# Oreoluwa-Se/Lidar-Imu-Slam

Measured on NVIDIA B200. Metric: deskew+ICP+GN-loop odometry throughput at 128k pts/scan, higher is better.
Workload: dtype f64

## Files before the change

### lidar-imu-slam_b200/csrc/voxelize.cu

```cuda
#include <algorithm>

#include "compact.cuh"
#include "grid_sync.cuh"
#include "imu_compensate.cuh"
#include "ops.cuh"
#include "voxel_map.cuh"

LIMU_TRACE_RING(limu_debug_trace_vox)

namespace limu {

constexpr int VX_BLOCK = 1024;
constexpr int VX_RUNS = 64;

struct VoxelizeArgs {
    const void *raw;
    const double *ts;
    int mode, stride, deskew;
    double twist[6];
    const double *twist_dev;
    int64_t n;
    double vs1, vs2;
    double *frame, *down, *src0;
    unsigned long long *keys1, *keys2;
    unsigned int *min1, *min2, *pslot1, *pslot2;
    unsigned long long *keys2_prev;
    unsigned int *min2_prev, *pslot2_prev;
    int *nd_prev, *nd_this;
    unsigned int mask1, mask2;
    int shift1, shift2;
    unsigned long long *tile1, *tile2;
    unsigned int epoch;
    int *counts;
    unsigned int *barrier;
    DevStatus *st;
    DevStatus *st_next;
};
struct VoxelizeImuArgs : VoxelizeArgs {
    ImuDeskew imu;
};

__device__ __forceinline__ unsigned int claim(unsigned long long *keys, unsigned int *minidx, int shift, unsigned int mask, const V3 &p, double vs,
                                              unsigned int index, DevStatus *st) {
    const int kx = vox_index(p.x, vs), ky = vox_index(p.y, vs), kz = vox_index(p.z, vs);
    if (!key_in_range(kx, ky, kz)) { st->key_range = 1; return PEND_NONE; }
    const unsigned long long key = pack_key(kx, ky, kz);
    unsigned int s = slot_of(key, shift);
    for (unsigned int probes = 0; probes <= mask; ++probes) {
        const unsigned long long cur = atomicCAS(&keys[s], KEY_EMPTY, key);
        if (cur == KEY_EMPTY || cur == key) { atomicMin(&minidx[s], index); return s; }
        s = (s + 1) & mask;
    }
    st->table_full = 1;
    return PEND_NONE;
}

__device__ __forceinline__ int block_exclusive_scan_count(int c, int *total, int *warp_sums ) {
    const int lane = threadIdx.x & 31, warp = threadIdx.x >> 5;
    int incl = c;
#pragma unroll
    for (int o = 1; o < 32; o <<= 1) { const int t = __shfl_up_sync(0xFFFFFFFFu, incl, o); if (lane >= o) incl += t; }
    if (lane == 31) warp_sums[warp] = incl;
    __syncthreads();
    if (warp == 0) {
        const int nw = (blockDim.x + 31) >> 5;
        const int v = lane < nw ? warp_sums[lane] : 0;
        int wi = v;
#pragma unroll
        for (int o = 1; o < 32; o <<= 1) { const int t = __shfl_up_sync(0xFFFFFFFFu, wi, o); if (lane >= o) wi += t; }
        warp_sums[lane] = wi - v;
        if (lane == 31) *total = wi;
    }
    __syncthreads();
    return warp_sums[warp] + incl - c;
}

template <int BLOCK>
__device__ __forceinline__ int tile_base(const unsigned long long *words, int tile, unsigned int epoch, int *ws ) {
    int part = 0;
    for (int b = threadIdx.x; b < tile; b += BLOCK) {
        unsigned long long w;
        do {
            asm volatile("ld.relaxed.gpu.global.u64 %0, [%1];" : "=l"(w) : "l"(words + b) : "memory");
        } while ((unsigned int)(w >> 32) != epoch);
        part += (int)(unsigned int)w;
    }
#pragma unroll
    for (int o = 16; o > 0; o >>= 1) part += __shfl_down_sync(0xFFFFFFFFu, part, o);
    __syncthreads();
    if ((threadIdx.x & 31) == 0) ws[threadIdx.x >> 5] = part;
    __syncthreads();
    int v = 0;
#pragma unroll
    for (int w = 0; w < BLOCK / 32; ++w) v += ws[w];
    __syncthreads();
    return v;
}
__device__ __forceinline__ void tile_publish(unsigned long long *word, unsigned int epoch, int count) {
    asm volatile("st.relaxed.gpu.global.u64 [%0], %1;" ::"l"(word), "l"(((unsigned long long)epoch << 32) | (unsigned int)count) : "memory");
}

#ifdef LIMU_ICP_PHASE_TIMING
__device__ unsigned long long g_vox_marks[8];
#define VX_MARK(k) do { if (blockIdx.x == 0 && threadIdx.x == 0) { unsigned long long _t; asm volatile("mov.u64 %0, %%globaltimer;" : "=l"(_t)); g_vox_marks[k] = _t; } } while (0)
#else
#define VX_MARK(k) do {} while (0)
#endif

__device__ __forceinline__ Pose deskew_motion(double t, const double *tw) {
    const double s = t - 0.5;
    double st[6];
#pragma unroll
    for (int k = 0; k < 6; ++k) st[k] = s * tw[k];
    return se3_exp(st);
}

template <bool IMU, class Args>
__device__ __forceinline__ void voxelize_body(const Args &A) {
    __shared__ int ws[32];
    __shared__ int total;
    GridSync gs{A.barrier, 0u, gridDim.x};
    const int64_t n = A.n;
    const int64_t gtid = (int64_t)blockIdx.x * VX_BLOCK + threadIdx.x, gthreads = (int64_t)gridDim.x * VX_BLOCK;
    const int ntiles = (int)((n + VX_BLOCK - 1) / VX_BLOCK);
    VX_MARK(0);
    LIMU_TRACE(10);
    {
        const int ndp = __ldcg(A.nd_prev);
        for (int64_t j = gtid; j < ndp; j += gthreads) {
            const unsigned int sl = __ldcg(A.pslot2_prev + j);
            if (sl != PEND_NONE) { A.keys2_prev[sl] = KEY_EMPTY; A.min2_prev[sl] = PEND_NONE; }
        }
    }
    if constexpr (IMU) {
        for (int64_t i = gtid; i < n; i += gthreads) {
            const unsigned char *r = static_cast<const unsigned char *>(A.raw) + (size_t)i * A.stride;
            const float *q = reinterpret_cast<const float *>(r);
            float xyz[3] = {q[0], q[1], q[2]};
            imu_deskew_point(A.imu.table, A.imu.M, i, imu_point_time(r, A.imu.toff), A.imu.rot_end, A.imu.pos_lidar_end, A.imu.p_il, xyz);
            const V3 p{(double)xyz[0], (double)xyz[1], (double)xyz[2]};
            A.frame[3 * i] = p.x; A.frame[3 * i + 1] = p.y; A.frame[3 * i + 2] = p.z;
            A.pslot1[i] = claim(A.keys1, A.min1, A.shift1, A.mask1, p, A.vs1, (unsigned int)i, A.st);
        }
    } else {
        __shared__ double tw[6];
        if (A.deskew && threadIdx.x == 0) {
#pragma unroll
            for (int k = 0; k < 6; ++k) tw[k] = A.twist_dev ? __ldcg(A.twist_dev + k) : A.twist[k];
        }
        __shared__ unsigned long long last_t[VX_BLOCK / 32];
        __shared__ Pose runs[VX_RUNS];
        const int lane = threadIdx.x & 31, warp = threadIdx.x >> 5;
        for (int tile = blockIdx.x; tile < ntiles; tile += gridDim.x) {
            const int64_t i = (int64_t)tile * VX_BLOCK + threadIdx.x;
            const bool live = i < n;
            double t = 0.0;
            if (live && A.deskew) t = A.mode == 0 ? (double)__ldg(reinterpret_cast<const float4 *>(A.raw) + i).w : A.mode == 1 ? A.ts[i] : 0.0;
            Pose T{};
            if (A.deskew) {
                const unsigned long long tb = (unsigned long long)__double_as_longlong(t);
                unsigned long long prev = __shfl_up_sync(0xFFFFFFFFu, tb, 1);
                if (lane == 31) last_t[warp] = tb;
                __syncthreads();
                if (lane == 0 && warp > 0) prev = last_t[warp - 1];
                const int head = live && (threadIdx.x == 0 || tb != prev);
                const int run = block_exclusive_scan_count(head, &total, ws) + head - 1;
                const bool table = total <= VX_RUNS;
                if (table && head) runs[run].qx = t;
                if (table) __syncthreads();
                const bool mine = table ? (int)threadIdx.x < total : live;
                if (mine) T = deskew_motion(table ? runs[threadIdx.x].qx : t, tw);
                if (table) {
                    if (mine) runs[threadIdx.x] = T;
                    __syncthreads();
                    if (live) T = runs[run];
                }
            }
            if (live) {
                V3 p;
                if (A.mode == 0) {
                    const float4 q = __ldg(reinterpret_cast<const float4 *>(A.raw) + i);
                    p = V3{(double)q.x, (double)q.y, (double)q.z};
                } else if (A.mode == 1) {
                    const float *q = reinterpret_cast<const float *>(static_cast<const unsigned char *>(A.raw) + (size_t)i * A.stride);
                    p = V3{(double)q[0], (double)q[1], (double)q[2]};
                } else {
                    const double *q = static_cast<const double *>(A.raw) + 3 * i;
                    p = V3{q[0], q[1], q[2]};
                }
                if (A.deskew) p = apply(T, p);
                A.frame[3 * i] = p.x; A.frame[3 * i + 1] = p.y; A.frame[3 * i + 2] = p.z;
                A.pslot1[i] = claim(A.keys1, A.min1, A.shift1, A.mask1, p, A.vs1, (unsigned int)i, A.st);
            }
        }
    }
    gs.sync();
    VX_MARK(1);
    LIMU_TRACE(11);
    for (int tile = blockIdx.x; tile < ntiles; tile += gridDim.x) {
        const int64_t i = (int64_t)tile * VX_BLOCK + threadIdx.x;
        int f = 0;
        if (i < n) { const unsigned int s = A.pslot1[i]; f = s != PEND_NONE && __ldcg(A.min1 + s) == (unsigned int)i; }
        const int r = block_exclusive_scan_count(f, &total, ws);
        if (threadIdx.x == 0) tile_publish(A.tile1 + tile, A.epoch, total);
        const int base = tile_base<VX_BLOCK>(A.tile1, tile, A.epoch, ws);
        if (f) {
            const int j = base + r;
            const V3 p{A.frame[3 * i], A.frame[3 * i + 1], A.frame[3 * i + 2]};
            A.down[3 * (size_t)j] = p.x; A.down[3 * (size_t)j + 1] = p.y; A.down[3 * (size_t)j + 2] = p.z;
            A.pslot2[j] = claim(A.keys2, A.min2, A.shift2, A.mask2, p, A.vs2, (unsigned int)j, A.st);
        }
        if (tile == ntiles - 1 && threadIdx.x == 0) { A.counts[0] = base + total; *A.nd_this = base + total; }
        __syncthreads();
    }
    if (ntiles == 0 && gtid == 0) { A.counts[0] = 0; *A.nd_this = 0; }
    gs.sync();
    VX_MARK(2);
    LIMU_TRACE(12);
    if (gtid == 0 && A.st_next) *A.st_next = DevStatus{0, 0, {0, 0}};
    for (int64_t i = gtid; i < n; i += gthreads) {
        const unsigned int sl = A.pslot1[i];
        if (sl != PEND_NONE) { A.keys1[sl] = KEY_EMPTY; A.min1[sl] = PEND_NONE; }
    }
    const int nd = __ldcg(A.counts);
    const int ntiles2 = (nd + VX_BLOCK - 1) / VX_BLOCK;
    for (int tile = blockIdx.x; tile < ntiles2; tile += gridDim.x) {
        const int j = tile * VX_BLOCK + (int)threadIdx.x;
        int f = 0;
        if (j < nd) { const unsigned int s = __ldcg(A.pslot2 + j); f = s != PEND_NONE && __ldcg(A.min2 + s) == (unsigned int)j; }
        const int r = block_exclusive_scan_count(f, &total, ws);
        if (threadIdx.x == 0) tile_publish(A.tile2 + tile, A.epoch, total);
        const int base = tile_base<VX_BLOCK>(A.tile2, tile, A.epoch, ws);
        if (f) {
            const size_t k = (size_t)(base + r);
            A.src0[3 * k] = __ldcg(A.down + 3 * (size_t)j); A.src0[3 * k + 1] = __ldcg(A.down + 3 * (size_t)j + 1); A.src0[3 * k + 2] = __ldcg(A.down + 3 * (size_t)j + 2);
        }
        if (tile == ntiles2 - 1 && threadIdx.x == 0) A.counts[1] = base + total;
        __syncthreads();
    }
    if (ntiles2 == 0 && gtid == 0) A.counts[1] = 0;
    __syncthreads();
    VX_MARK(3);
    LIMU_TRACE(13);
    if (threadIdx.x == 0) {
        __threadfence();
        if (atomicAdd(A.barrier + 1, 1u) == gridDim.x - 1) { A.barrier[0] = 0u; A.barrier[1] = 0u; __threadfence(); }
    }
}
static __global__ void __launch_bounds__(VX_BLOCK, 1) k_voxelize_full(const VoxelizeArgs A) { voxelize_body<false>(A); }
static __global__ void __maxnreg__(48) k_voxelize_lean(const VoxelizeArgs A) { voxelize_body<false>(A); }
static __global__ void __launch_bounds__(VX_BLOCK, 1) k_voxelize_imu_full(const VoxelizeImuArgs A) { voxelize_body<true>(A); }
static __global__ void __maxnreg__(48) k_voxelize_imu_lean(const VoxelizeImuArgs A) { voxelize_body<true>(A); }

static __global__ void k_gate(const unsigned int *flag, unsigned int seq) {
    unsigned long long t0, t1;
    asm volatile("mov.u64 %0, %%globaltimer;" : "=l"(t0));
    for (unsigned int spins = 1;; ++spins) {
        unsigned int v;
        asm volatile("ld.acquire.gpu.global.u32 %0, [%1];" : "=r"(v) : "l"(flag) : "memory");
        if ((int)(v - seq) >= 0) break;
        if ((spins & 1023u) == 0u) {
            asm volatile("mov.u64 %0, %%globaltimer;" : "=l"(t1));
            if (t1 - t0 > 5000000000ull) break;
        }
    }
    LIMU_TRACE(30);
}
int gate_device(cudaStream_t s, const unsigned int *flag, unsigned int seq) {
    static bool hinted = false;
    if (!hinted) {
        if (cudaFuncSetAttribute(k_gate, cudaFuncAttributePreferredSharedMemoryCarveout, cudaSharedmemCarveoutMaxShared) != cudaSuccess) (void)cudaGetLastError();
        hinted = true;
    }
    k_gate<<<1, 1, 0, s>>>(flag, seq);
    LIMU_LAUNCHED();
    return LIMU_OK;
}

#ifdef LIMU_ICP_PHASE_TIMING
extern "C" int limu_debug_vox_marks(double out[8]) {
    unsigned long long h[8];
    if (cudaMemcpyFromSymbol(h, g_vox_marks, sizeof h) != cudaSuccess) return -1;
    for (int k = 0; k < 8; ++k) out[k] = (double)h[k];
    return 0;
}
#endif

static int g_vx_blocks_per_sm = 0;

static int64_t pow2_slots(int64_t n) { int64_t p = 1024; while (p < 2 * n) p <<= 1; return p; }

int voxelize_device(limu_ctx *c, VoxelizeScratch &sc, const Scan &scan, int deskew, const double *twist_host, double v, double *frame_dev, double *down_dev,
                    double *src0_dev, int *counts_dev, const double *twist_dev, DevStatus *own_status, int *status_used, cudaStream_t stream, bool beside) {
    if (!stream) stream = c->stream;
    if (scan.layout == SCAN_IMU && !scan.imu) { set_error("voxelize_device: an IMU scan without IMU deskew arguments"); return LIMU_ERR_INVALID; }
    const int64_t n = scan.n;
    if (n <= 0) {
        LIMU_CUDA_TRY(cudaMemsetAsync(counts_dev, 0, 2 * sizeof(int), stream));
        if (own_status) {
            const int w = sc.st_word;
            sc.st_word = (w + 1) % 3;
            LIMU_CUDA_TRY(cudaMemsetAsync(own_status + w, 0, sizeof(DevStatus), stream));
            LIMU_CUDA_TRY(cudaMemsetAsync(own_status + sc.st_word, 0, sizeof(DevStatus), stream));
            if (status_used) *status_used = w;
        } else if (status_used) *status_used = 0;
        return LIMU_OK;
    }
    if (g_vx_blocks_per_sm == 0) {
        int b = 0;
        LIMU_CUDA_TRY(cudaOccupancyMaxActiveBlocksPerMultiprocessor(&b, k_voxelize_full, VX_BLOCK, 0));
        g_vx_blocks_per_sm = std::max(1, std::min(b, 1024 / VX_BLOCK));
    }
    const int64_t C1 = pow2_slots(n), C2 = pow2_slots(n);
    int lg = 0;
    while ((int64_t(1) << lg) < C1) ++lg;
    const int ntiles = div_up(n, VX_BLOCK);
    {
        bool reset = false;
        if (C1 > sc.cap_slots) {
            int64_t cap = sc.cap_slots ? sc.cap_slots : 1024;
            while (cap < C1) cap <<= 1;
            LIMU_TRY(sc.table.reserve((size_t)cap * 12 * 3, stream));
            sc.cap_slots = cap;
            reset = true;
        }
        const void *before = sc.pslot.p;
        LIMU_TRY(sc.pslot.reserve((size_t)n * 4 * 3, stream));
        if (sc.pslot.p != before) reset = true;
        sc.pslot_n = (int64_t)(sc.pslot.bytes / 12);
        before = sc.tiles.p;
        LIMU_TRY(sc.tiles.reserve((size_t)ntiles * 16 + 128, stream));
        if (sc.tiles.p != before) reset = true;
        if (reset) {
            LIMU_CUDA_TRY(cudaMemsetAsync(sc.table.p, 0xFF, (size_t)sc.cap_slots * 12 * 3, stream));
            LIMU_CUDA_TRY(cudaMemsetAsync(sc.tiles.p, 0, sc.tiles.bytes, stream));
        }
    }
    const int par = sc.parity;
    sc.parity ^= 1;
    VoxelizeImuArgs X;
    VoxelizeArgs &A = X;
    A.raw = scan.ptr; A.ts = scan.ts; A.mode = scan.layout; A.stride = scan.stride; A.deskew = deskew; A.n = n;
    for (int k = 0; k < 6; ++k) A.twist[k] = (deskew && twist_host) ? twist_host[k] : 0.0;
    A.twist_dev = deskew ? twist_dev : nullptr;
    A.vs1 = v * 0.5; A.vs2 = v * 1.5;
    A.frame = frame_dev; A.down = down_dev; A.src0 = src0_dev;
    {
        unsigned char *base = sc.table.as<unsigned char>();
        const size_t tb = (size_t)sc.cap_slots * 12;
        auto keys_of = [&](int t) { return reinterpret_cast<unsigned long long *>(base + tb * t); };
        auto min_of = [&](int t) { return reinterpret_cast<unsigned int *>(base + tb * t + (size_t)sc.cap_slots * 8); };
        A.keys1 = keys_of(0); A.min1 = min_of(0);
        A.keys2 = keys_of(1 + par); A.min2 = min_of(1 + par);
        A.keys2_prev = keys_of(1 + (par ^ 1)); A.min2_prev = min_of(1 + (par ^ 1));
    }
    A.mask1 = (unsigned int)(C1 - 1); A.mask2 = (unsigned int)(C2 - 1); A.shift1 = A.shift2 = 64 - lg;
    A.pslot1 = sc.pslot.as<unsigned int>();
    A.pslot2 = A.pslot1 + sc.pslot_n * (1 + par);
    A.pslot2_prev = A.pslot1 + sc.pslot_n * (1 + (par ^ 1));
    A.barrier = sc.tiles.as<unsigned int>();
    A.nd_this = sc.tiles.as<int>() + 4 + par;
    A.nd_prev = sc.tiles.as<int>() + 4 + (par ^ 1);
    A.tile1 = reinterpret_cast<unsigned long long *>(sc.tiles.as<int>() + 16); A.tile2 = A.tile1 + ntiles;
    if (++sc.epoch == 0u) sc.epoch = 1u;
    A.epoch = sc.epoch;
    A.counts = counts_dev;
    const int w = sc.st_word;
    if (own_status) sc.st_word = (w + 1) % 3;
    A.st = own_status ? own_status + w : c->d_status;
    A.st_next = own_status ? own_status + sc.st_word : nullptr;
    if (status_used) *status_used = w;
    const int grid = (int)std::min<int64_t>(ntiles, beside ? (int64_t)std::max(1, c->sm_count - GATE_SLACK_SMS) : (int64_t)c->sm_count * g_vx_blocks_per_sm);
    void *args[] = {&A};
    const void *fn = beside ? (const void *)k_voxelize_lean : (const void *)k_voxelize_full;
    if (scan.layout == SCAN_IMU) {
        const ImuCall &a = *scan.imu;
        X.imu.table = scan.imu_table; X.imu.M = a.M; X.imu.toff = a.toff;
        memcpy(X.imu.rot_end, a.rot_end, sizeof a.rot_end); memcpy(X.imu.pos_lidar_end, a.pos_lidar_end, sizeof a.pos_lidar_end); memcpy(X.imu.p_il, a.p_il, sizeof a.p_il);
        args[0] = &X;
        fn = beside ? (const void *)k_voxelize_imu_lean : (const void *)k_voxelize_imu_full;
    }
    LIMU_CUDA_TRY(cudaLaunchCooperativeKernel(fn, dim3(grid), dim3(VX_BLOCK), args, 0, stream));
    LIMU_LAUNCHED();
    return LIMU_OK;
}

}
```

Before: 10340.

## Fuse both voxel-grid claims into one pass with warp-level key dedup

Each point now claims its fine and coarse voxel slots in the first pass. Nesting of the coarse key in the fine key (coarse = fine/3) is checked, and when it holds for every point, both compactions run in a single scan with packed 16-bit counters. This removes a grid sync, the second claim pass and the per-point table clearing, which moves into the next call via double-buffered tables. __match_any_sync dedup cuts atomicCAS contention on shared keys. The cost is twice the table and pslot memory, a fallback path when keys are not nested, and a tile count packed into 16 bits, which assumes block-level counts stay small.

```diff
diff --git a/lidar-imu-slam_b200/csrc/voxelize.cu b/lidar-imu-slam_b200/csrc/voxelize.cu
--- a/lidar-imu-slam_b200/csrc/voxelize.cu
+++ b/lidar-imu-slam_b200/csrc/voxelize.cu
@@ -23,10 +23,11 @@
     double vs1, vs2;
     double *frame, *down, *src0;
     unsigned long long *keys1, *keys2;
-    unsigned int *min1, *min2, *pslot1, *pslot2;
-    unsigned long long *keys2_prev;
-    unsigned int *min2_prev, *pslot2_prev;
-    int *nd_prev, *nd_this;
+    unsigned int *min1, *min2;
+    unsigned int *pslot1, *pslot2;
+    unsigned long long *keys1_prev, *keys2_prev;
+    unsigned int *min1_prev, *min2_prev, *pslot1_prev, *pslot2_prev;
+    int *won_prev, *won_this;
     unsigned int mask1, mask2;
     int shift1, shift2;
     unsigned long long *tile1, *tile2;
@@ -40,19 +41,44 @@
     ImuDeskew imu;
 };
 
+__device__ __forceinline__ unsigned int claim_from(unsigned long long *keys, unsigned int *minidx, unsigned int mask, unsigned int s, unsigned long long cur,
+                                                   unsigned long long key, unsigned int index, DevStatus *st) {
+    for (unsigned int probes = 0;;) {
+        if (cur == KEY_EMPTY || cur == key) { atomicMin(&minidx[s], index); return s; }
+        if (++probes > mask) { st->table_full = 1; return PEND_NONE; }
+        s = (s + 1) & mask;
+        cur = atomicCAS(&keys[s], KEY_EMPTY, key);
+    }
+}
 __device__ __forceinline__ unsigned int claim(unsigned long long *keys, unsigned int *minidx, int shift, unsigned int mask, const V3 &p, double vs,
                                               unsigned int index, DevStatus *st) {
     const int kx = vox_index(p.x, vs), ky = vox_index(p.y, vs), kz = vox_index(p.z, vs);
     if (!key_in_range(kx, ky, kz)) { st->key_range = 1; return PEND_NONE; }
     const unsigned long long key = pack_key(kx, ky, kz);
-    unsigned int s = slot_of(key, shift);
-    for (unsigned int probes = 0; probes <= mask; ++probes) {
-        const unsigned long long cur = atomicCAS(&keys[s], KEY_EMPTY, key);
-        if (cur == KEY_EMPTY || cur == key) { atomicMin(&minidx[s], index); return s; }
-        s = (s + 1) & mask;
-    }
-    st->table_full = 1;
-    return PEND_NONE;
+    const unsigned int s = slot_of(key, shift);
+    return claim_from(keys, minidx, mask, s, atomicCAS(&keys[s], KEY_EMPTY, key), key, index, st);
+}
+template <class Args>
+__device__ __forceinline__ void claim_both(const Args &A, const V3 &p, unsigned int index) {
+    const int ax = vox_index(p.x, A.vs1), ay = vox_index(p.y, A.vs1), az = vox_index(p.z, A.vs1);
+    const bool in1 = key_in_range(ax, ay, az);
+    if (!in1) A.st->key_range = 1;
+    const int bx = vox_index(p.x, A.vs2), by = vox_index(p.y, A.vs2), bz = vox_index(p.z, A.vs2);
+    const bool nested = bx == ax / 3 && by == ay / 3 && bz == az / 3;
+    if (in1 && !nested) A.barrier[2] = 1u;
+    const bool in2 = in1 && nested;
+    const unsigned long long k1 = in1 ? pack_key(ax, ay, az) : KEY_EMPTY, k2 = in2 ? pack_key(bx, by, bz) : KEY_EMPTY;
+    const unsigned int active = __activemask();
+    const int lead1 = __ffs(__match_any_sync(active, k1)) - 1, lead2 = __ffs(__match_any_sync(active, k2)) - 1;
+    const int lane = threadIdx.x & 31;
+    const bool claims1 = in1 && lane == lead1, claims2 = in2 && lane == lead2;
+    unsigned int s1 = slot_of(k1, A.shift1), s2 = slot_of(k2, A.shift2);
+    const unsigned long long c1 = claims1 ? atomicCAS(&A.keys1[s1], KEY_EMPTY, k1) : 0ull;
+    const unsigned long long c2 = claims2 ? atomicCAS(&A.keys2[s2], KEY_EMPTY, k2) : 0ull;
+    s1 = claims1 ? claim_from(A.keys1, A.min1, A.mask1, s1, c1, k1, index, A.st) : PEND_NONE;
+    s2 = claims2 ? claim_from(A.keys2, A.min2, A.mask2, s2, c2, k2, index, A.st) : PEND_NONE;
+    A.pslot1[index] = __shfl_sync(active, s1, lead1);
+    A.pslot2[index] = __shfl_sync(active, s2, lead2);
 }
 
 __device__ __forceinline__ int block_exclusive_scan_count(int c, int *total, int *warp_sums ) {
@@ -76,21 +102,21 @@
 }
 
 template <int BLOCK>
-__device__ __forceinline__ int tile_base(const unsigned long long *words, int tile, unsigned int epoch, int *ws ) {
-    int part = 0;
+__device__ __forceinline__ unsigned long long tile_base(const unsigned long long *words, int tile, unsigned int epoch) {
+    __shared__ unsigned long long ws[BLOCK / 32];
+    unsigned long long part = 0;
     for (int b = threadIdx.x; b < tile; b += BLOCK) {
         unsigned long long w;
         do {
             asm volatile("ld.relaxed.gpu.global.u64 %0, [%1];" : "=l"(w) : "l"(words + b) : "memory");
         } while ((unsigned int)(w >> 32) != epoch);
-        part += (int)(unsigned int)w;
+        part += (w & 0xFFFFull) | (w & 0xFFFF0000ull) << 16;
     }
 #pragma unroll
     for (int o = 16; o > 0; o >>= 1) part += __shfl_down_sync(0xFFFFFFFFu, part, o);
-    __syncthreads();
     if ((threadIdx.x & 31) == 0) ws[threadIdx.x >> 5] = part;
     __syncthreads();
-    int v = 0;
+    unsigned long long v = 0;
 #pragma unroll
     for (int w = 0; w < BLOCK / 32; ++w) v += ws[w];
     __syncthreads();
@@ -126,8 +152,12 @@
     VX_MARK(0);
     LIMU_TRACE(10);
     {
-        const int ndp = __ldcg(A.nd_prev);
+        const int ndp = __ldcg(A.won_prev), nsp = __ldcg(A.won_prev + 1);
         for (int64_t j = gtid; j < ndp; j += gthreads) {
+            const unsigned int sl = __ldcg(A.pslot1_prev + j);
+            if (sl != PEND_NONE) { A.keys1_prev[sl] = KEY_EMPTY; A.min1_prev[sl] = PEND_NONE; }
+        }
+        for (int64_t j = gtid; j < nsp; j += gthreads) {
             const unsigned int sl = __ldcg(A.pslot2_prev + j);
             if (sl != PEND_NONE) { A.keys2_prev[sl] = KEY_EMPTY; A.min2_prev[sl] = PEND_NONE; }
         }
@@ -140,7 +170,7 @@
             imu_deskew_point(A.imu.table, A.imu.M, i, imu_point_time(r, A.imu.toff), A.imu.rot_end, A.imu.pos_lidar_end, A.imu.p_il, xyz);
             const V3 p{(double)xyz[0], (double)xyz[1], (double)xyz[2]};
             A.frame[3 * i] = p.x; A.frame[3 * i + 1] = p.y; A.frame[3 * i + 2] = p.z;
-            A.pslot1[i] = claim(A.keys1, A.min1, A.shift1, A.mask1, p, A.vs1, (unsigned int)i, A.st);
+            claim_both(A, p, (unsigned int)i);
         }
     } else {
         __shared__ double tw[6];
@@ -190,61 +220,103 @@
                 }
                 if (A.deskew) p = apply(T, p);
                 A.frame[3 * i] = p.x; A.frame[3 * i + 1] = p.y; A.frame[3 * i + 2] = p.z;
-                A.pslot1[i] = claim(A.keys1, A.min1, A.shift1, A.mask1, p, A.vs1, (unsigned int)i, A.st);
+                claim_both(A, p, (unsigned int)i);
             }
         }
     }
     gs.sync();
     VX_MARK(1);
     LIMU_TRACE(11);
-    for (int tile = blockIdx.x; tile < ntiles; tile += gridDim.x) {
-        const int64_t i = (int64_t)tile * VX_BLOCK + threadIdx.x;
-        int f = 0;
-        if (i < n) { const unsigned int s = A.pslot1[i]; f = s != PEND_NONE && __ldcg(A.min1 + s) == (unsigned int)i; }
-        const int r = block_exclusive_scan_count(f, &total, ws);
-        if (threadIdx.x == 0) tile_publish(A.tile1 + tile, A.epoch, total);
-        const int base = tile_base<VX_BLOCK>(A.tile1, tile, A.epoch, ws);
-        if (f) {
-            const int j = base + r;
-            const V3 p{A.frame[3 * i], A.frame[3 * i + 1], A.frame[3 * i + 2]};
-            A.down[3 * (size_t)j] = p.x; A.down[3 * (size_t)j + 1] = p.y; A.down[3 * (size_t)j + 2] = p.z;
+    if (gtid == 0 && A.st_next) *A.st_next = DevStatus{0, 0, {0, 0}};
+    if (__ldcg(A.barrier + 2) == 0u) {
+        for (int tile = blockIdx.x; tile < ntiles; tile += gridDim.x) {
+            const int64_t i = (int64_t)tile * VX_BLOCK + threadIdx.x;
+            unsigned int s1 = PEND_NONE, s2 = PEND_NONE;
+            int f1 = 0, f2 = 0;
+            if (i < n) {
+                s1 = A.pslot1[i];
+                f1 = s1 != PEND_NONE && __ldcg(A.min1 + s1) == (unsigned int)i;
+                if (f1) { s2 = A.pslot2[i]; f2 = s2 != PEND_NONE && __ldcg(A.min2 + s2) == (unsigned int)i; }
+            }
+            const int r = block_exclusive_scan_count(f1 | f2 << 16, &total, ws);
+            if (threadIdx.x == 0) tile_publish(A.tile1 + tile, A.epoch, total);
+            const unsigned long long base = tile_base<VX_BLOCK>(A.tile1, tile, A.epoch);
+            const int b1 = (int)(unsigned int)base, b2 = (int)(base >> 32);
+            if (f1) {
+                const size_t j = (size_t)(b1 + (r & 0xFFFF));
+                const V3 p{A.frame[3 * i], A.frame[3 * i + 1], A.frame[3 * i + 2]};
+                A.down[3 * j] = p.x; A.down[3 * j + 1] = p.y; A.down[3 * j + 2] = p.z;
+                A.pslot1[j] = s1;
+                if (f2) {
+                    const size_t k = (size_t)(b2 + (r >> 16));
+                    A.src0[3 * k] = p.x; A.src0[3 * k + 1] = p.y; A.src0[3 * k + 2] = p.z;
+                    A.pslot2[k] = s2;
+                }
+            }
+            if (tile == ntiles - 1 && threadIdx.x == 0) {
+                const int nd = b1 + (total & 0xFFFF), ns = b2 + (total >> 16);
+                A.counts[0] = nd; A.counts[1] = ns; A.won_this[0] = nd; A.won_this[1] = ns;
+            }
+            __syncthreads();
+        }
+    } else {
+        for (int tile = blockIdx.x; tile < ntiles; tile += gridDim.x) {
+            const int64_t i = (int64_t)tile * VX_BLOCK + threadIdx.x;
+            unsigned int s1 = PEND_NONE;
+            int f = 0;
+            if (i < n) {
+                s1 = A.pslot1[i];
+                f = s1 != PEND_NONE && __ldcg(A.min1 + s1) == (unsigned int)i;
+                const unsigned int s2 = A.pslot2[i];
+                if (s2 != PEND_NONE) { A.keys2[s2] = KEY_EMPTY; A.min2[s2] = PEND_NONE; }
+            }
+            const int r = block_exclusive_scan_count(f, &total, ws);
+            if (threadIdx.x == 0) tile_publish(A.tile1 + tile, A.epoch, total);
+            const int base = (int)(unsigned int)tile_base<VX_BLOCK>(A.tile1, tile, A.epoch);
+            if (f) {
+                const size_t j = (size_t)(base + r);
+                A.down[3 * j] = A.frame[3 * i]; A.down[3 * j + 1] = A.frame[3 * i + 1]; A.down[3 * j + 2] = A.frame[3 * i + 2];
+                A.pslot1[j] = s1;
+            }
+            if (tile == ntiles - 1 && threadIdx.x == 0) { A.counts[0] = base + total; A.won_this[0] = base + total; }
+            __syncthreads();
+        }
+        gs.sync();
+        VX_MARK(3);
+        LIMU_TRACE(12);
+        const int nd = __ldcg(A.counts);
+        for (int64_t j = gtid; j < nd; j += gthreads) {
+            const V3 p{__ldcg(A.down + 3 * j), __ldcg(A.down + 3 * j + 1), __ldcg(A.down + 3 * j + 2)};
             A.pslot2[j] = claim(A.keys2, A.min2, A.shift2, A.mask2, p, A.vs2, (unsigned int)j, A.st);
         }
-        if (tile == ntiles - 1 && threadIdx.x == 0) { A.counts[0] = base + total; *A.nd_this = base + total; }
-        __syncthreads();
-    }
-    if (ntiles == 0 && gtid == 0) { A.counts[0] = 0; *A.nd_this = 0; }
-    gs.sync();
+        gs.sync();
+        VX_MARK(4);
+        LIMU_TRACE(14);
+        const int ntiles2 = (nd + VX_BLOCK - 1) / VX_BLOCK;
+        for (int tile = blockIdx.x; tile < ntiles2; tile += gridDim.x) {
+            const int j = tile * VX_BLOCK + (int)threadIdx.x;
+            unsigned int s = PEND_NONE;
+            int f = 0;
+            if (j < nd) { s = __ldcg(A.pslot2 + j); f = s != PEND_NONE && __ldcg(A.min2 + s) == (unsigned int)j; }
+            const int r = block_exclusive_scan_count(f, &total, ws);
+            if (threadIdx.x == 0) tile_publish(A.tile2 + tile, A.epoch, total);
+            const int base = (int)(unsigned int)tile_base<VX_BLOCK>(A.tile2, tile, A.epoch);
+            if (f) {
+                const size_t k = (size_t)(base + r);
+                A.src0[3 * k] = __ldcg(A.down + 3 * (size_t)j); A.src0[3 * k + 1] = __ldcg(A.down + 3 * (size_t)j + 1); A.src0[3 * k + 2] = __ldcg(A.down + 3 * (size_t)j + 2);
+                A.pslot2[k] = s;
+            }
+            if (tile == ntiles2 - 1 && threadIdx.x == 0) { A.counts[1] = base + total; A.won_this[1] = base + total; }
+            __syncthreads();
+        }
+        if (ntiles2 == 0 && gtid == 0) { A.counts[1] = 0; A.won_this[1] = 0; }
+    }
+    __syncthreads();
     VX_MARK(2);
-    LIMU_TRACE(12);
-    if (gtid == 0 && A.st_next) *A.st_next = DevStatus{0, 0, {0, 0}};
-    for (int64_t i = gtid; i < n; i += gthreads) {
-        const unsigned int sl = A.pslot1[i];
-        if (sl != PEND_NONE) { A.keys1[sl] = KEY_EMPTY; A.min1[sl] = PEND_NONE; }
-    }
-    const int nd = __ldcg(A.counts);
-    const int ntiles2 = (nd + VX_BLOCK - 1) / VX_BLOCK;
-    for (int tile = blockIdx.x; tile < ntiles2; tile += gridDim.x) {
-        const int j = tile * VX_BLOCK + (int)threadIdx.x;
-        int f = 0;
-        if (j < nd) { const unsigned int s = __ldcg(A.pslot2 + j); f = s != PEND_NONE && __ldcg(A.min2 + s) == (unsigned int)j; }
-        const int r = block_exclusive_scan_count(f, &total, ws);
-        if (threadIdx.x == 0) tile_publish(A.tile2 + tile, A.epoch, total);
-        const int base = tile_base<VX_BLOCK>(A.tile2, tile, A.epoch, ws);
-        if (f) {
-            const size_t k = (size_t)(base + r);
-            A.src0[3 * k] = __ldcg(A.down + 3 * (size_t)j); A.src0[3 * k + 1] = __ldcg(A.down + 3 * (size_t)j + 1); A.src0[3 * k + 2] = __ldcg(A.down + 3 * (size_t)j + 2);
-        }
-        if (tile == ntiles2 - 1 && threadIdx.x == 0) A.counts[1] = base + total;
-        __syncthreads();
-    }
-    if (ntiles2 == 0 && gtid == 0) A.counts[1] = 0;
-    __syncthreads();
-    VX_MARK(3);
     LIMU_TRACE(13);
     if (threadIdx.x == 0) {
         __threadfence();
-        if (atomicAdd(A.barrier + 1, 1u) == gridDim.x - 1) { A.barrier[0] = 0u; A.barrier[1] = 0u; __threadfence(); }
+        if (atomicAdd(A.barrier + 1, 1u) == gridDim.x - 1) { A.barrier[0] = 0u; A.barrier[1] = 0u; A.barrier[2] = 0u; __threadfence(); }
     }
 }
 static __global__ void __launch_bounds__(VX_BLOCK, 1) k_voxelize_full(const VoxelizeArgs A) { voxelize_body<false>(A); }
@@ -320,19 +392,19 @@
         if (C1 > sc.cap_slots) {
             int64_t cap = sc.cap_slots ? sc.cap_slots : 1024;
             while (cap < C1) cap <<= 1;
-            LIMU_TRY(sc.table.reserve((size_t)cap * 12 * 3, stream));
+            LIMU_TRY(sc.table.reserve((size_t)cap * 12 * 4, stream));
             sc.cap_slots = cap;
             reset = true;
         }
         const void *before = sc.pslot.p;
-        LIMU_TRY(sc.pslot.reserve((size_t)n * 4 * 3, stream));
+        LIMU_TRY(sc.pslot.reserve((size_t)n * 4 * 4, stream));
         if (sc.pslot.p != before) reset = true;
-        sc.pslot_n = (int64_t)(sc.pslot.bytes / 12);
+        sc.pslot_n = (int64_t)(sc.pslot.bytes / 16);
         before = sc.tiles.p;
         LIMU_TRY(sc.tiles.reserve((size_t)ntiles * 16 + 128, stream));
         if (sc.tiles.p != before) reset = true;
         if (reset) {
-            LIMU_CUDA_TRY(cudaMemsetAsync(sc.table.p, 0xFF, (size_t)sc.cap_slots * 12 * 3, stream));
+            LIMU_CUDA_TRY(cudaMemsetAsync(sc.table.p, 0xFF, (size_t)sc.cap_slots * 12 * 4, stream));
             LIMU_CUDA_TRY(cudaMemsetAsync(sc.tiles.p, 0, sc.tiles.bytes, stream));
         }
     }
@@ -350,17 +422,18 @@
         const size_t tb = (size_t)sc.cap_slots * 12;
         auto keys_of = [&](int t) { return reinterpret_cast<unsigned long long *>(base + tb * t); };
         auto min_of = [&](int t) { return reinterpret_cast<unsigned int *>(base + tb * t + (size_t)sc.cap_slots * 8); };
-        A.keys1 = keys_of(0); A.min1 = min_of(0);
-        A.keys2 = keys_of(1 + par); A.min2 = min_of(1 + par);
-        A.keys2_prev = keys_of(1 + (par ^ 1)); A.min2_prev = min_of(1 + (par ^ 1));
+        A.keys1 = keys_of(2 * par); A.min1 = min_of(2 * par);
+        A.keys2 = keys_of(2 * par + 1); A.min2 = min_of(2 * par + 1);
+        A.keys1_prev = keys_of(2 * (par ^ 1)); A.min1_prev = min_of(2 * (par ^ 1));
+        A.keys2_prev = keys_of(2 * (par ^ 1) + 1); A.min2_prev = min_of(2 * (par ^ 1) + 1);
     }
     A.mask1 = (unsigned int)(C1 - 1); A.mask2 = (unsigned int)(C2 - 1); A.shift1 = A.shift2 = 64 - lg;
-    A.pslot1 = sc.pslot.as<unsigned int>();
-    A.pslot2 = A.pslot1 + sc.pslot_n * (1 + par);
-    A.pslot2_prev = A.pslot1 + sc.pslot_n * (1 + (par ^ 1));
+    unsigned int *pslot = sc.pslot.as<unsigned int>();
+    A.pslot1 = pslot + sc.pslot_n * (2 * par); A.pslot2 = pslot + sc.pslot_n * (2 * par + 1);
+    A.pslot1_prev = pslot + sc.pslot_n * (2 * (par ^ 1)); A.pslot2_prev = pslot + sc.pslot_n * (2 * (par ^ 1) + 1);
     A.barrier = sc.tiles.as<unsigned int>();
-    A.nd_this = sc.tiles.as<int>() + 4 + par;
-    A.nd_prev = sc.tiles.as<int>() + 4 + (par ^ 1);
+    A.won_this = sc.tiles.as<int>() + 4 + 2 * par;
+    A.won_prev = sc.tiles.as<int>() + 4 + 2 * (par ^ 1);
     A.tile1 = reinterpret_cast<unsigned long long *>(sc.tiles.as<int>() + 16); A.tile2 = A.tile1 + ntiles;
     if (++sc.epoch == 0u) sc.epoch = 1u;
     A.epoch = sc.epoch;
```

New measurement: 10460 (median of 6 runs). 1.01x the previous value.
